# multimodallearning/convexAdam

Measured on AMD Instinct MI355X. Metric: volume-pairs/sec (160x192x224 MIND convex+Adam(80it)), higher is better.
Workload: dtype f32

## Files before the change

convexadam_amd/csrc/adam.hip:

```cpp
#include <math.h>

#include "cvx_common.h"

namespace cvx {

constexpr int BT_Z = 8, BT_Y = 8, BT_X = 32, BT_NT = 512, BT_PX = 48;

template <int PASS, bool BACKWARD, bool ADAM>
__device__ __forceinline__ void box_pass(const float* __restrict__ src, int sy, float* __restrict__ dst, int dz, int dy,
                                         int gz0, int gy0, int x0, int h, int w, int d, float* __restrict__ gout,
                                         float* __restrict__ P, float* __restrict__ m, float* __restrict__ v, AdamConsts ac,
                                         float* __restrict__ gsave) {
    constexpr int NP = 20 - PASS, C0 = 4 + PASS, SH = PASS - 1;
    const int nr = dz * dy * NP;
    for (int r = threadIdx.x; r < nr; r += BT_NT) {
        const int p = r % NP, row = r / NP;
        const int y = row % dy, z = row / dy;
        const int c = C0 + 2 * p;
        const float* win = src + ((z + 1) * sy + (y + 1)) * BT_PX + (c - 1 + SH);
        f32x2 s = {0.0f, 0.0f};
#pragma unroll
        for (int a = -1; a <= 1; ++a)
#pragma unroll
            for (int b = -1; b <= 1; ++b) {
// ... 86 lines not shown
__global__ __launch_bounds__(256) void k_adam_update(const float* __restrict__ G, float* __restrict__ P, float* __restrict__ m,
                                                     float* __restrict__ v, size_t n, AdamConsts ac) {
    const size_t i = (size_t)blockIdx.x * blockDim.x + threadIdx.x;
    if (i >= n) return;
    const float g = G[i];
    const float mo = m[i];
    const float mm = __builtin_fmaf(ac.w1, g - mo, mo);
    float vv = v[i] * ac.b2;
    vv = __builtin_fmaf(ac.omb2 * g, g, vv);
    const float den = fdiv(adam_sqrt(vv, ac.sqrt_tbl), ac.bc2s) + 1e-8f;
    P[i] = P[i] + fdiv(ac.neg_step * mm, den);
    m[i] = mm;
    v[i] = vv;
}

static int launch_box3x3(const float* in, float* out, int h, int w, int d, bool backward, float* P, float* m, float* v,
                         AdamConsts ac, float* gsave, hipStream_t s) {
    const bool force_tiled = options().box_tiled != 0;
    if (!force_tiled && (backward ? (out || P) && box3_tile_supported(in, out, h, w, d, P, m, v, gsave) : box3_tile_fwd_supported(in, out, h, w, d))) {
        long long ft = backward ? options().box_bwd_tile : options().box_fwd_tile;
        if (ft < 0) ft = box3_march_supported(d) ? box3_tile_fwd_auto(h, w, d) : 2000;
        if (ft >= 1000) return launch_box3_tile(in, out, h, w, d, (int)ft, backward, P, m, v, ac, gsave, s);
    }
    if (!force_tiled && box3_march_supported(d)) return launch_box3_march(in, out, h, w, d, backward, P, m, v, ac, gsave, s);
    const int nb = cdiv(d, BT_X) * cdiv(w, BT_Y) * cdiv(h, BT_Z) * 3;
    if (!backward) hipLaunchKernelGGL((k_box3x3<false, false>), dim3(nb), dim3(BT_NT), 0, s, in, out, h, w, d, P, m, v, ac, gsave);
    else if (!P) hipLaunchKernelGGL((k_box3x3<true, false>), dim3(nb), dim3(BT_NT), 0, s, in, out, h, w, d, P, m, v, ac, gsave);
    else hipLaunchKernelGGL((k_box3x3<true, true>), dim3(nb), dim3(BT_NT), 0, s, in, out, h, w, d, P, m, v, ac, gsave);
    return check_last("box3x3");
}

}

using namespace cvx;

extern "C" size_t cvx_adam_workspace_bytes(int C, int h, int w, int d) {
    const size_t V = (size_t)h * w * d, CP = (size_t)(C + 3) / 4 * 4;
    return 3 * (256 + sizeof(float) * 3 * V) + 2 * (256 + sizeof(float) * CP * (V + 1)) + 256;
// ... 103 lines not shown
    }

    const float nH = (float)((int64_t)3 * (h - 1) * w * d), nW = (float)((int64_t)3 * h * (w - 1) * d),
                nD = (float)((int64_t)3 * h * w * (d - 1));
    const float cH = lambda_weight / nH, cW = lambda_weight / nW, cD = lambda_weight / nD;
    const float gsc = ((1.0f / (float)V) * cost_scale) / (float)C;
    int snap = 0;
    for (int it = 0; it < niter; ++it) {
        int rc;
        const int step = step0 + it + 1;
        const double beta1 = 0.9, beta2 = 0.999;
        const double bc1 = 1.0 - pow(beta1, (double)step), bc2 = 1.0 - pow(beta2, (double)step);
        const AdamConsts ac = {(float)(1.0 - beta1), (float)beta2, (float)(1.0 - beta2), (float)sqrt(bc2), (float)(-(1.0 / bc1)), adam_sqrt_table()};
        if (fast == 2 && fused) { if ((rc = launch_box3_fast(P, U, h, w, d, nullptr, nullptr, nullptr, 1.0, 1.0, nullptr, s))) return rc; }
        else if (fast == 2 && sm->kind == 0) { if ((rc = launch_boxchain_fast(P, U, h, w, d, *sm, false, s))) return rc; }
        else if (fused) { if ((rc = launch_box3x3(P, U, h, w, d, false, nullptr, nullptr, nullptr, ac, nullptr, s))) return rc; }
        else if ((rc = launch_smoother(P, U, t1, 3, h, w, d, *sm, false, s))) return rc;
        profile_mark_kernel("adam.forward_boxes", s);
        const bool last = it == niter - 1;
        if (!(last && !keep_state && !grad_out)) {
        float* gsave = (grad_out && it == niter - 1) ? grad_out : nullptr;
        if (fast) {
            if ((rc = launch_warp_grad_fast(Fcl, Mcl, C, h, w, d, U, base_h, base_w, base_d, gsc, cH, cW, cD, gU, f16_features, s))) return rc;
            profile_mark_kernel("adam.warp_gradient", s);
            if (fused) { if ((rc = launch_box3_fast(gU, nullptr, h, w, d, P, m, v, bc1, bc2, gsave, s))) return rc; }
            else {
                if (sm->kind == 0) { if ((rc = launch_boxchain_fast(gU, t2, h, w, d, *sm, true, s))) return rc; }
                else if ((rc = launch_smoother(gU, t2, t1, 3, h, w, d, *sm, true, s))) return rc;
                if ((rc = launch_adam_update_fast(t2, P, m, v, 3 * V, bc1, bc2, s))) return rc;
                if (gsave) (void)hipMemcpyAsync(gsave, t2, sizeof(float) * 3 * V, hipMemcpyDeviceToDevice, s);
            }
        } else {
        if ((rc = launch_warp_grad(Fcl, Mcl, C, h, w, d, U, base_h, base_w, base_d, gsc, cH, cW, cD, gU, f16_features, s))) return rc;
        profile_mark_kernel("adam.warp_gradient", s);
        if (fused) { if ((rc = launch_box3x3(gU, nullptr, h, w, d, true, P, m, v, ac, gsave, s))) return rc; }
        else {
            if ((rc = launch_smoother(gU, t2, t1, 3, h, w, d, *sm, true, s))) return rc;
            hipLaunchKernelGGL(k_adam_update, dim3((unsigned)cdiv64((int64_t)(3 * V), 256)), dim3(256), 0, s, t2, P, m, v, 3 * V, ac);
            if (gsave) (void)hipMemcpyAsync(gsave, t2, sizeof(float) * 3 * V, hipMemcpyDeviceToDevice, s);
        }
        }
        }
        if (!(last && !keep_state && !grad_out)) profile_mark_kernel("adam.adjoint_update", s);
        while (snap < n_snap && snapshot_iters_host[snap] == it + 1) {
            (void)hipMemcpyAsync(snapshots + (size_t)snap * 3 * V, U, sizeof(float) * 3 * V, hipMemcpyDeviceToDevice, s);
            ++snap;
        }
    }
    return check_last("adam_run");
}
// ... 1 lines not shown
```

convexadam_amd/csrc/api.hip:

```cpp
#include <math.h>
#include <stdlib.h>
#include <string.h>
#include <new>

#include "cvx_common.h"

namespace cvx {

static thread_local char g_err[512] = "";

void set_error(const char* fmt, ...) {
    va_list ap;
    va_start(ap, fmt);
    vsnprintf(g_err, sizeof(g_err), fmt, ap);
    va_end(ap);
}
int fail(int code, const char* fmt, ...) {
    va_list ap;
    va_start(ap, fmt);
    vsnprintf(g_err, sizeof(g_err), fmt, ap);
    va_end(ap);
    return code;
}
int check_last(const char* what) {
// ... 9 lines not shown

}
struct cvx_context {
    cvx::Options opt;
    unsigned* sqrt_tbl = nullptr;
    unsigned char* exp_tbl = nullptr;
    unsigned exp_first = 0, exp_count = 0;
    int tbl_device = -1;
};
namespace cvx {
static Options env_options() {
    return {env_ll("CVX_MIND_TILED", 0),   env_ll("CVX_MIND_OVERLAP", 0),  env_ll("CVX_MM_TX", 0),        env_ll("CVX_MM_SLOTS", 512),          env_ll("CVX_BOX_TILED", 0),
            env_ll("CVX_NO_PRUNE", 0),     env_ll("CVX_CORR_UNFUSED", 0), env_ll("CVX_CORR_FUSED_ALL", 0), env_ll("CVX_PRUNE_STREAM_ABOVE", -1), env_ll("CVX_CF_CENSUS", 0), env_ll("CVX_CF_PRIO", 136),
            env_ll("CVX_WARP_FLAT", 0),    env_ll("CVX_BOX_YT", 8),       env_ll("CVX_BOX_WG_TARGET", 0),
            env_ll("CVX_BOX_XSPLIT", -1),  env_ll("CVX_BOX_CPT", 4),      env_ll("CVX_BOX_UNEVEN", 200), env_ll("CVX_BOX_ADAM_ROLE", 0), env_ll("CVX_BOX_DPP", 0),      env_ll("CVX_BOX_PK", 0),       env_ll("CVX_BOX_PRIO", 0),     env_ll("CVX_LABEL_POW_BLOCK", 32), 0,                             env_ll("CVX_MIND_MEAN_THREADS", 0),
            env_ll("CVX_EDT_SEQUENTIAL", 0), env_ll("CVX_WARP_OCTANT", 4), env_ll("CVX_BOX_FWD_TILE", -1), env_ll("CVX_BOX_BWD_TILE", -1), env_ll("CVX_BOX_WALK", 1), env_ll("CVX_CORR_DUAL", 0), env_ll("CVX_PRUNE_REFINE", 1), env_ll("CVX_MIND_RECORDS", 1), env_ll("CVX_RESIZE_UP2", 1), env_ll("CVX_MIND_BLOCKED", 1), env_ll("CVX_CORR_CERT", 1), env_ll("CVX_CC_DEBUG", 0), env_ll("CVX_IC_FUSED", 0), env_ll("CVX_MIND_SINGLE", 0), env_ll("CVX_MS_ZLEN", 0), env_ll("CVX_CF_MAP", 1), env_ll("CVX_CERT_UNFUSED", 0), env_ll("CVX_FBOX_TILE", 0)};
}
static cvx_context& default_context() {
    static cvx_context c = [] { cvx_context d; d.opt = env_options(); return d; }();
    return c;
}
static thread_local cvx_context* t_bound = nullptr;
static cvx_context& current_context() { return t_bound ? *t_bound : default_context(); }
Options& options() { return current_context().opt; }
const unsigned* adam_sqrt_table() { return current_context().sqrt_tbl; }
ExpTable mind_exp_table() {
    const cvx_context& c = current_context();
    return {c.exp_tbl, c.exp_first, c.exp_tbl ? c.exp_count : 0u};
}
ContextScope::ContextScope(const cvx_context* c) : prev_(t_bound), active_(c != nullptr) {
    if (active_) t_bound = const_cast<cvx_context*>(c);
// ... 31 lines not shown
    *slot = p;
    return CVX_OK;
}
constexpr size_t kSqrtTableBytes = ((size_t)(1u << 24) + (1u << 23)) / 4;

__global__ __launch_bounds__(256) void k_expf(const float* __restrict__ x, float* __restrict__ out, size_t n) {
    for (size_t i = (size_t)blockIdx.x * blockDim.x + threadIdx.x; i < n; i += (size_t)gridDim.x * blockDim.x) out[i] = cvx_expf(x[i]);
}
struct OptName { const char* name; long long Options::*field; };
static const OptName kOptNames[] = {{"mind_tiled", &Options::mind_tiled},     {"mind_overlap", &Options::mind_overlap},   {"mm_tx", &Options::mm_tx},
                                    {"mm_slots", &Options::mm_slots},         {"box_tiled", &Options::box_tiled},
                                    {"no_prune", &Options::no_prune},         {"corr_unfused", &Options::corr_unfused}, {"corr_fused_all", &Options::corr_fused_all},
                                    {"prune_stream_above", &Options::prune_stream_above}, {"cf_census", &Options::cf_census}, {"cf_prio", &Options::cf_prio},
                                    {"warp_flat", &Options::warp_flat},       {"box_yt", &Options::box_yt},             {"box_wg_target", &Options::box_wg_target},
                                    {"box_xsplit", &Options::box_xsplit},     {"box_cpt", &Options::box_cpt},           {"box_uneven", &Options::box_uneven},     {"box_adam_role", &Options::box_adam_role}, {"box_dpp", &Options::box_dpp},           {"box_pk", &Options::box_pk},             {"box_prio", &Options::box_prio},         {"label_pow_block", &Options::label_pow_block}, {"census_ptr", &Options::census_ptr},     {"mind_mean_threads", &Options::mind_mean_threads},
                                    {"edt_sequential", &Options::edt_sequential}, {"warp_octant", &Options::warp_octant}, {"box_fwd_tile", &Options::box_fwd_tile}, {"box_bwd_tile", &Options::box_bwd_tile}, {"box_walk", &Options::box_walk}, {"corr_dual", &Options::corr_dual}, {"prune_refine", &Options::prune_refine}, {"mind_records", &Options::mind_records}, {"resize_up2", &Options::resize_up2}, {"mind_blocked", &Options::mind_blocked}, {"corr_cert", &Options::corr_cert}, {"cc_debug", &Options::cc_debug}, {"ic_fused", &Options::ic_fused}, {"mind_single", &Options::mind_single}, {"ms_zlen", &Options::ms_zlen}, {"cf_map", &Options::cf_map}, {"cert_unfused", &Options::cert_unfused}, {"fbox_tile", &Options::fbox_tile}};

}

static int set_option_of(cvx_context& c, const char* name, long long value) {
    for (const auto& o : cvx::kOptNames)
        if (name && strcmp(name, o.name) == 0) {
            if (strcmp(name, "box_xsplit") == 0 && value > 32) return cvx::fail(CVX_ERR_INVALID_ARG, "box_xsplit %lld: at most 32 x tiles", value);
            c.opt.*(o.field) = value;
            return CVX_OK;
        }
    return cvx::fail(CVX_ERR_INVALID_ARG, "cvx_set_option: unknown option '%s'", name ? name : "(null)");
}
static long long get_option_of(const cvx_context& c, const char* name) {
    for (const auto& o : cvx::kOptNames)
        if (name && strcmp(name, o.name) == 0) return c.opt.*(o.field);
// ... 89 lines not shown
```

convexadam_amd/csrc/boxtile.hip:

```cpp
#include "cvx_common.h"

namespace cvx {

namespace {

constexpr unsigned BT_OOB = 0x80000000u;

struct BTWin { float w[3][6]; };

template <bool F, bool M, bool P>
__device__ __forceinline__ void bt_accum(const BTWin& t, float (&mid)[4], float (&pre)[4], float (&fin)[4]) {
    float f[4], m[4], p[4];
#pragma unroll
    for (int j = 0; j < 4; ++j) { f[j] = mid[j]; m[j] = pre[j]; p[j] = 0.0f; }
#pragma unroll
    for (int i = 0; i < 3; ++i)
#pragma unroll
        for (int j = 0; j < 4; ++j) {
            if (F) { f[j] += t.w[i][j]; f[j] += t.w[i][j + 1]; f[j] += t.w[i][j + 2]; }
            if (M) { m[j] += t.w[i][j]; m[j] += t.w[i][j + 1]; m[j] += t.w[i][j + 2]; }
            if (P) { p[j] += t.w[i][j]; p[j] += t.w[i][j + 1]; p[j] += t.w[i][j + 2]; }
        }
#pragma unroll
    for (int j = 0; j < 4; ++j) { fin[j] = f[j]; mid[j] = m[j]; pre[j] = p[j]; }
// ... 35 lines not shown
        bt_accum<true, false, false>(A, mid, pre, fin);
        emit(L - 1, fin);
    } else {
        load(L + 1, B);
        prep(A);
        bt_accum<true, true, false>(A, mid, pre, fin);
        emit(L - 2, fin);
        prep(B);
        bt_accum<true, false, false>(B, mid, pre, fin);
        emit(L - 1, fin);
    }
}

}

template <int TZ, int TY, int TXQ, int NW, int WPS, bool BACKWARD, bool ADAM>
__global__ __launch_bounds__(64 * NW, WPS) void k_box3_tile(const float* __restrict__ in, float* __restrict__ out, int h, int w, int d,
                                                           int ntz, int nty, int ntx, int ntiles, int NS1, int NS2, int NS3, FastDiv dvz, FastDiv dvx, FastDiv dvy,
                                                           FastDiv dn1, FastDiv dn2, FastDiv dn3, float* __restrict__ P, float* __restrict__ m, float* __restrict__ v, AdamConsts ac,
                                                           float* __restrict__ gsave) {
    constexpr int TX = 4 * TXQ, RS = TX + 4;
    constexpr int Z1 = TZ + 4, Y1 = TY + 4, Z2 = TZ + 2, Y2 = TY + 2;
    constexpr int SLOTS = NW * 4;
    static_assert(TXQ + 2 <= 16, "a row of quads must fit 16 lanes");
    __shared__ __attribute__((aligned(16))) float S[Z1 * Y1 * RS + Z2 * Y2 * RS + 8];
    float* S1 = S;
    float* S2 = S + Z1 * Y1 * RS;
    const int per_xcd = (int)(gridDim.x >> 3);
    const int bid = __builtin_amdgcn_readfirstlane((int)blockIdx.x);
    const int b = (bid & 7) * per_xcd + (bid >> 3);
    if (b >= ntiles) return;
// ... 18 lines not shown
            const int yy = gy - 1 + i;
            ro[i] = (qin && yy >= 0 && yy < w) ? (unsigned)(yy * d + gx) * 4u : BT_OOB;
        }
        const int zin0 = z0 - 3 + p0;
        auto load = [&](int n, BTWin& t) {
            const int z = zin0 + n;
            const bool zok = z >= 0 && z < h;
            const unsigned zo = (unsigned)(zok ? z : 0) * (unsigned)wd * 4u;
#pragma unroll
            for (int i = 0; i < 3; ++i) {
                const float4 a = buffer_load16(ir, (zok && ro[i] != BT_OOB) ? ro[i] + zo : BT_OOB, 0);
                t.w[i][1] = a.x; t.w[i][2] = a.y; t.w[i][3] = a.z; t.w[i][4] = a.w;
            }
        };
        auto prep = [&](BTWin& t) {
            if (BACKWARD) {
#pragma unroll
                for (int i = 0; i < 3; ++i)
#pragma unroll
                    for (int j = 1; j <= 4; ++j) t.w[i][j] = t.w[i][j] == 0.0f ? t.w[i][j] : div_exact<27>(t.w[i][j]);
            }
#pragma unroll
            for (int i = 0; i < 3; ++i) {
                t.w[i][0] = __int_as_float(__builtin_amdgcn_update_dpp(0, __float_as_int(t.w[i][4]), 0x111, 0xf, 0xf, true));
                t.w[i][5] = __int_as_float(__builtin_amdgcn_update_dpp(0, __float_as_int(t.w[i][1]), 0x101, 0xf, 0xf, true));
            }
        };
        const bool rowin = qin && gy >= 0 && gy < w;
        float* dst = S1 + (p0 * Y1 + r) * RS + 4 * q - 2;
        auto emit = [&](int k, const float (&fin)[4]) {
            const int z = z0 - 2 + p0 + k;
// ... 55 lines not shown
                for (int i = 0; i < 3; ++i) {
                    const float* rp = src + (n * Y2 + i) * RS;
                    const f32x4 a = lds_load4(rp);
                    const f32x2 e = lds_load2(rp + 4);
                    t.w[i][0] = a.x; t.w[i][1] = a.y; t.w[i][2] = a.z; t.w[i][3] = a.w; t.w[i][4] = e.x; t.w[i][5] = e.y;
                }
            };
            const size_t o0 = ((size_t)(z0 + p0) * w + gy) * d + gx;
            auto emit = [&](int k, const float (&fin)[4]) {
                if (z0 + p0 + k >= h) return;
                const size_t o = o0 + (size_t)k * wd;
                if (!BACKWARD) {
                    *reinterpret_cast<float4*>(oc + o) = make_float4(div_exact<27>(fin[0]), div_exact<27>(fin[1]), div_exact<27>(fin[2]), div_exact<27>(fin[3]));
                } else if (!ADAM) {
                    *reinterpret_cast<float4*>(oc + o) = make_float4(fin[0], fin[1], fin[2], fin[3]);
                } else {
                    float* Pc = P + (size_t)c * V + o; float* mc = m + (size_t)c * V + o; float* vc = v + (size_t)c * V + o;
                    const float4 p4 = *reinterpret_cast<const float4*>(Pc), m4 = *reinterpret_cast<const float4*>(mc), v4 = *reinterpret_cast<const float4*>(vc);
                    float pp[4] = {p4.x, p4.y, p4.z, p4.w}, mm[4] = {m4.x, m4.y, m4.z, m4.w}, vv[4] = {v4.x, v4.y, v4.z, v4.w};
#pragma unroll
                    for (int j = 0; j < 4; ++j) adam_update(fin[j], pp[j], mm[j], vv[j], ac);
                    *reinterpret_cast<float4*>(Pc) = make_float4(pp[0], pp[1], pp[2], pp[3]);
                    *reinterpret_cast<float4*>(mc) = make_float4(mm[0], mm[1], mm[2], mm[3]);
                    *reinterpret_cast<float4*>(vc) = make_float4(vv[0], vv[1], vv[2], vv[3]);
                    if (gsave) *reinterpret_cast<float4*>(gsave + (size_t)c * V + o) = make_float4(fin[0], fin[1], fin[2], fin[3]);
                }
            };
            bt_walk(L, load, [](BTWin&) {}, emit);
        }
    }
}

bool box3_tile_supported(const float* in, const float* out, int h, int w, int d, const float* P, const float* m, const float* v, const float* gsave) {
    auto al = [](const void* p) { return (reinterpret_cast<uintptr_t>(p) & 15) == 0; };
    return (d % 4 == 0) && al(in) && al(out) && al(P) && al(m) && al(v) && al(gsave) && in != out && (size_t)h * w * d * 4 < ((size_t)1 << 31);
}
bool box3_tile_fwd_supported(const float* in, const float* out, int h, int w, int d) { return out && box3_tile_supported(in, out, h, w, d, nullptr, nullptr, nullptr, nullptr); }

template <int TZ, int TY, int TXQ, int NW, int WPS>
static int launch_tile_t(const float* in, float* out, int h, int w, int d, int ns1, int ns2, int ns3, bool backward, float* P, float* m, float* v,
                         AdamConsts ac, float* gsave, hipStream_t s) {
    const int ntz = cdiv(h, TZ), nty = cdiv(w, TY), ntx = cdiv(d, 4 * TXQ);
    const int ntiles = 3 * ntz * nty * ntx;
    const unsigned nb = (unsigned)((ntiles + 7) / 8 * 8);
    auto clampns = [](int ns, int planes) { return ns < 1 ? 1 : (ns > planes / 2 ? planes / 2 : ns); };
    const int a1 = clampns(ns1, TZ + 4), a2 = clampns(ns2, TZ + 2), a3 = clampns(ns3, TZ);
#define CVX_BT_LAUNCH(B, A) hipLaunchKernelGGL((k_box3_tile<TZ, TY, TXQ, NW, WPS, B, A>), dim3(nb), dim3(64 * NW), 0, s, in, out, h, w, d, ntz, nty, ntx, ntiles, a1, a2, a3, fastdiv_make(ntz), fastdiv_make(ntx), fastdiv_make(nty), fastdiv_make(a1), fastdiv_make(a2), fastdiv_make(a3), P, m, v, ac, gsave)
    if (!backward) CVX_BT_LAUNCH(false, false);
    else if (!P) CVX_BT_LAUNCH(true, false);
    else CVX_BT_LAUNCH(true, true);
#undef CVX_BT_LAUNCH
    return check_last("box3_tile");
}

int launch_box3_tile(const float* in, float* out, int h, int w, int d, int variant, bool backward, float* P, float* m, float* v, AdamConsts ac,
                     float* gsave, hipStream_t s) {
    const int kind = variant / 1000, ns = variant % 1000;
    int ns1 = ns / 100, ns2 = (ns / 10) % 10, ns3 = ns % 10;
    if (kind == 1) {
        if (!ns) { ns1 = 5; ns2 = 3; ns3 = 4; }
        return launch_tile_t<12, 8, 14, 8, 4>(in, out, h, w, d, ns1, ns2, ns3, backward, P, m, v, ac, gsave, s);
    }
    if (!ns) { ns1 = 4; ns2 = 3; ns3 = 4; }
    return launch_tile_t<12, 16, 14, 16, 4>(in, out, h, w, d, ns1, ns2, ns3, backward, P, m, v, ac, gsave, s);
}
int launch_box3_tile_fwd(const float* in, float* out, int h, int w, int d, int variant, hipStream_t s) {
    return launch_box3_tile(in, out, h, w, d, variant, false, nullptr, nullptr, nullptr, AdamConsts{}, nullptr, s);
}

int box3_tile_fwd_auto(int h, int w, int d) {
    const int n2 = 3 * cdiv(h, 12) * cdiv(w, 16) * cdiv(d, 56);
    return n2 >= 192 ? 2000 : 0;
}

}
```

convexadam_amd/csrc/cvx_common.h:

```cpp
#pragma once
#include <hip/hip_runtime.h>
#include <stdint.h>
#include <stdio.h>
#include <stdarg.h>

#include <mutex>

#include "convexadam_hip.h"

namespace cvx {

void set_error(const char* fmt, ...);
int fail(int code, const char* fmt, ...);
int check_last(const char* what);

#define CVX_REQUIRE(cond, ...)                                      \
    do {                                                            \
        if (!(cond)) return ::cvx::fail(CVX_ERR_INVALID_ARG, __VA_ARGS__); \
    } while (0)

static inline hipStream_t as_stream(void* s) { return reinterpret_cast<hipStream_t>(s); }
static inline size_t align_up(size_t v, size_t a) { return (v + a - 1) / a * a; }
static inline int cdiv(int a, int b) { return (a + b - 1) / b; }
static inline int64_t cdiv64(int64_t a, int64_t b) { return (a + b - 1) / b; }
// ... 54 lines not shown
    long long box_bwd_tile;
    long long box_walk;
    long long corr_dual;
    long long prune_refine;
    long long mind_records;
    long long resize_up2;
    long long mind_blocked;
    long long corr_cert;
    long long cc_debug;
    long long ic_fused;
    long long mind_single;
    long long ms_zlen;
    long long cf_map;
    long long cert_unfused;
    long long fbox_tile;
};
Options& options();
const unsigned* adam_sqrt_table();
class ContextScope {
public:
    explicit ContextScope(const cvx_context* c);
    ~ContextScope();
    ContextScope(const ContextScope&) = delete;
    ContextScope& operator=(const ContextScope&) = delete;
private:
    void* prev_;
    bool active_;
};

#ifdef CVX_RACE_JITTER
// ... 231 lines not shown
size_t corr_certify_workspace_bytes(int C, int h, int w, int d, int hw, bool plain = false);
int corr_certified_argmin(const float* ssdu, const float* fix, const float* mov, int C, int h, int w, int d, int hw, int64_t* argmin,
                          void* workspace, size_t workspace_bytes, hipStream_t s);
int coupled_convex_cert_impl(const float* ssduA, const float* fixA, const float* movA, float* outA, void* wsA, const float* ssduB, const float* fixB,
                             const float* movB, float* outB, void* wsB, const float* mesh, int C, int h, int w, int d, int hw, size_t workspace_bytes,
                             hipStream_t s, int stage = 0);
bool corr_use_unfused(int C, int h, int w, int d, int hw, bool variant);
bool box3_march_supported(int d);
int launch_box3_march(const float* in, float* out, int h, int w, int d, bool backward, float* P, float* m, float* v,
                      AdamConsts ac, float* gsave, hipStream_t s);
bool box3_tile_fwd_supported(const float* in, const float* out, int h, int w, int d);
int launch_box3_tile_fwd(const float* in, float* out, int h, int w, int d, int variant, hipStream_t s);
int box3_tile_fwd_auto(int h, int w, int d);
bool box3_tile_supported(const float* in, const float* out, int h, int w, int d, const float* P, const float* m, const float* v, const float* gsave);
int launch_box3_tile(const float* in, float* out, int h, int w, int d, int variant, bool backward, float* P, float* m, float* v, AdamConsts ac,
                     float* gsave, hipStream_t s);
int launch_to_chunked(const float* in, int C, size_t V, float* out, bool half, hipStream_t s);
int launch_warp_grad(const float* Fcl, const float* Mcl, int C, int h, int w, int d, const float* U, const float* bh,
                     const float* bw, const float* bd, float gsc, float cH, float cW, float cD, float* gU, bool half, hipStream_t s);
int launch_warp_grad_fast(const float* Fcl, const float* Mcl, int C, int h, int w, int d, const float* U, const float* bh,
                          const float* bw, const float* bd, float gsc, float cH, float cW, float cD, float* gU, bool half, hipStream_t s);
int launch_box3_fast(const float* in, float* out, int h, int w, int d, float* P, float* m, float* v, double bc1, double bc2,
                     float* gsave, hipStream_t s);
bool boxchain_fast_supported(const cvx_smoother& sm, int h, int w, int d);
int launch_boxchain_fast(const float* in, float* out, int h, int w, int d, const cvx_smoother& sm, bool reverse, hipStream_t s);
int launch_adam_update_fast(const float* G, float* P, float* m, float* v, size_t n, double bc1, double bc2, hipStream_t s);

}
```

convexadam_amd/csrc/warp.hip:

```cpp
#include "cvx_common.h"

namespace cvx {

__global__ __launch_bounds__(256) void k_to_chunked(const float* __restrict__ in, int C, size_t V, float* __restrict__ out) {
    const size_t p = (size_t)blockIdx.x * blockDim.x + threadIdx.x;
    if (p > V) return;
    const int c0 = 4 * (int)blockIdx.y;
    float4 r = make_float4(0.f, 0.f, 0.f, 0.f);
    if (p < V) {
        const float* src = in + (size_t)c0 * V + p;
        r.x = src[0];
        if (c0 + 1 < C) r.y = src[V];
        if (c0 + 2 < C) r.z = src[2 * V];
        if (c0 + 3 < C) r.w = src[3 * V];
    }
    reinterpret_cast<float4*>(out)[(size_t)blockIdx.y * (V + 1) + p] = r;
}

typedef _Float16 h16x4 __attribute__((ext_vector_type(4)));
__global__ __launch_bounds__(256) void k_to_chunked_h(const float* __restrict__ in, int C, size_t V, uint2* __restrict__ out) {
    const size_t p = (size_t)blockIdx.x * blockDim.x + threadIdx.x;
    if (p > V) return;
    const int c0 = 4 * (int)blockIdx.y;
    float4 r = make_float4(0.f, 0.f, 0.f, 0.f);
    if (p < V) {
        const float* src = in + (size_t)c0 * V + p;
        r.x = src[0];
        if (c0 + 1 < C) r.y = src[V];
        if (c0 + 2 < C) r.z = src[2 * V];
        if (c0 + 3 < C) r.w = src[3 * V];
    }
    const h16x4 o = {(_Float16)r.x, (_Float16)r.y, (_Float16)r.z, (_Float16)r.w};
    out[(size_t)blockIdx.y * (V + 1) + p] = __builtin_bit_cast(uint2, o);
}
__device__ __forceinline__ float4 buffer_load8h(__amdgpu_buffer_rsrc_t rsrc, unsigned lane_off, unsigned uni_off) {
    const h16x4 v = __builtin_bit_cast(h16x4, __builtin_amdgcn_raw_buffer_load_b64(rsrc, (int)lane_off, (int)uni_off, 0));
    return make_float4((float)v.x, (float)v.y, (float)v.z, (float)v.w);
}

template <bool BUF, bool HALF = false>
__global__ __launch_bounds__(256) void k_warp_grad(const float* __restrict__ F2, const float* __restrict__ M2, int C, int CP,
                                                   int h, int w, int d, const float* __restrict__ U,
                                                   const float* __restrict__ bh, const float* __restrict__ bw,
                                                   const float* __restrict__ bd, float gsc, float cH, float cW, float cD,
                                                   float* __restrict__ gU, unsigned long long* __restrict__ census, FastDiv dx, FastDiv dy,
                                                   float sc0, float sc1, float sc2) {
    const size_t V = (size_t)h * w * d;
    if (census && threadIdx.x == 0) {
        census[4 * blockIdx.x] = __builtin_amdgcn_s_memrealtime();
        census[4 * blockIdx.x + 3] = __builtin_amdgcn_s_getreg((4 << 0) | (0 << 6) | (31 << 11)) | ((unsigned long long)__builtin_amdgcn_s_getreg((20 << 0) | (0 << 6) | (31 << 11)) << 32);
    }
    const int ntx = (d + 15) / 16, nty = (w + 3) / 4, ntz = (h + 3) / 4;
    const int per_xcd = (int)(gridDim.x >> 3);
    const int bid = __builtin_amdgcn_readfirstlane((int)blockIdx.x);
    const int tile = (bid & 7) * per_xcd + (bid >> 3);
// ... 16 lines not shown
    unsigned off[8];
    off[0] = (zin0 && yin0 && xin0) ? (unsigned)(r00 + x0) * REC : zero_rec; off[1] = (zin0 && yin0 && xin1) ? (unsigned)(r00 + x1) * REC : zero_rec;
    off[2] = (zin0 && yin1 && xin0) ? (unsigned)(r01 + x0) * REC : zero_rec; off[3] = (zin0 && yin1 && xin1) ? (unsigned)(r01 + x1) * REC : zero_rec;
    off[4] = (zin1 && yin0 && xin0) ? (unsigned)(r10 + x0) * REC : zero_rec; off[5] = (zin1 && yin0 && xin1) ? (unsigned)(r10 + x1) * REC : zero_rec;
    off[6] = (zin1 && yin1 && xin0) ? (unsigned)(r11 + x0) * REC : zero_rec; off[7] = (zin1 && yin1 && xin1) ? (unsigned)(r11 + x1) * REC : zero_rec;
    const float wgt[8] = {t.tnw, t.tne, t.tsw, t.tse, t.bnw, t.bne, t.bsw, t.bse};
    const float ax[8] = {fy1 - t.iy, fy1 - t.iy, t.iy - fy0, t.iy - fy0, fy1 - t.iy, fy1 - t.iy, t.iy - fy0, t.iy - fy0};
    const float bx[8] = {fz1 - t.iz, fz1 - t.iz, fz1 - t.iz, fz1 - t.iz, t.iz - fz0, t.iz - fz0, t.iz - fz0, t.iz - fz0};
    const float ay[8] = {fx1 - t.ix, t.ix - fx0, fx1 - t.ix, t.ix - fx0, fx1 - t.ix, t.ix - fx0, fx1 - t.ix, t.ix - fx0};
    const float bz[8] = {fy1 - t.iy, fy1 - t.iy, t.iy - fy0, t.iy - fy0, fy1 - t.iy, fy1 - t.iy, t.iy - fy0, t.iy - fy0};
    float gix = 0.f, giy = 0.f, giz = 0.f;
    const unsigned foff = p * REC;
    const unsigned chunk_bytes = (unsigned)(V + 1) * REC;
    const __amdgpu_buffer_rsrc_t mr = __builtin_amdgcn_make_buffer_rsrc(const_cast<float*>(M2), 0, (int)(chunk_bytes * (unsigned)(CP / 4)), 0x00020000);
    const __amdgpu_buffer_rsrc_t fr = __builtin_amdgcn_make_buffer_rsrc(const_cast<float*>(F2), 0, (int)(chunk_bytes * (unsigned)(CP / 4)), 0x00020000);
    unsigned coff = 0;
    for (int c0 = 0; c0 < CP / 4; ++c0, coff += chunk_bytes) {
        float vv[8][4], fv[4];
#pragma unroll
        for (int k = 0; k < 8; ++k) {
            const float4 q = HALF ? buffer_load8h(mr, off[k], coff) : BUF ? buffer_load16(mr, off[k], coff) : *reinterpret_cast<const float4*>(reinterpret_cast<const char*>(M2) + (size_t)c0 * chunk_bytes + off[k]);
            vv[k][0] = q.x; vv[k][1] = q.y; vv[k][2] = q.z; vv[k][3] = q.w;
        }
        const float4 fq = HALF ? buffer_load8h(fr, foff, coff) : BUF ? buffer_load16(fr, foff, coff) : *reinterpret_cast<const float4*>(reinterpret_cast<const char*>(F2) + (size_t)c0 * chunk_bytes + foff);
        fv[0] = fq.x; fv[1] = fq.y; fv[2] = fq.z; fv[3] = fq.w;
#pragma unroll
        for (int j = 0; j < 4; ++j) {
            float wv = 0.0f;
#pragma unroll
            for (int k = 0; k < 8; ++k) wv += vv[k][j] * wgt[k];
// ... 1 lines not shown
            const float gOut = gsc * (2.0f * df);
            gix -= vv[0][j] * ax[0] * bx[0] * gOut; giy -= vv[0][j] * ay[0] * bx[0] * gOut; giz -= vv[0][j] * ay[0] * bz[0] * gOut;
            gix += vv[1][j] * ax[1] * bx[1] * gOut; giy -= vv[1][j] * ay[1] * bx[1] * gOut; giz -= vv[1][j] * ay[1] * bz[1] * gOut;
            gix -= vv[2][j] * ax[2] * bx[2] * gOut; giy += vv[2][j] * ay[2] * bx[2] * gOut; giz -= vv[2][j] * ay[2] * bz[2] * gOut;
            gix += vv[3][j] * ax[3] * bx[3] * gOut; giy += vv[3][j] * ay[3] * bx[3] * gOut; giz -= vv[3][j] * ay[3] * bz[3] * gOut;
            gix -= vv[4][j] * ax[4] * bx[4] * gOut; giy -= vv[4][j] * ay[4] * bx[4] * gOut; giz += vv[4][j] * ay[4] * bz[4] * gOut;
            gix += vv[5][j] * ax[5] * bx[5] * gOut; giy -= vv[5][j] * ay[5] * bx[5] * gOut; giz += vv[5][j] * ay[5] * bz[5] * gOut;
            gix -= vv[6][j] * ax[6] * bx[6] * gOut; giy += vv[6][j] * ay[6] * bx[6] * gOut; giz += vv[6][j] * ay[6] * bz[6] * gOut;
            gix += vv[7][j] * ax[7] * bx[7] * gOut; giy += vv[7][j] * ay[7] * bx[7] * gOut; giz += vv[7][j] * ay[7] * bz[7] * gOut;
        }
    }
    float g[3];
    g[0] = fdiv(((float)h / 2.0f) * giz, sc0);
    g[1] = fdiv(((float)w / 2.0f) * giy, sc1);
    g[2] = fdiv(((float)d / 2.0f) * gix, sc2);
    const unsigned sH = (unsigned)(w * d);
    const unsigned pxp = x < d - 1 ? p + 1 : p, pxm = x > 0 ? p - 1 : p, pzp = z < h - 1 ? p + sH : p, pzm = z > 0 ? p - sH : p,
                   pyp = y < w - 1 ? p + (unsigned)d : p, pym = y > 0 ? p - (unsigned)d : p;
    float nb[3][6];
    const __amdgpu_buffer_rsrc_t ur = __builtin_amdgcn_make_buffer_rsrc(const_cast<float*>(U), 0, (int)(12u * (unsigned)V), 0x00020000);
    const unsigned nboff[6] = {4u * pxp, 4u * pxm, 4u * pzp, 4u * pzm, 4u * pyp, 4u * pym};
#pragma unroll
    for (int a = 0; a < 3; ++a)
#pragma unroll
        for (int k = 0; k < 6; ++k) nb[a][k] = __builtin_bit_cast(float, __builtin_amdgcn_raw_buffer_load_b32(ur, (int)nboff[k], (int)(4u * (unsigned)V) * a, 0));
    const float uc3[3] = {uH, uW, uD};
#pragma unroll
    for (int a = 0; a < 3; ++a) {
        const float uc = uc3[a];
        float acc = g[a], t;
        t = acc + -(cD * (2.0f * (nb[a][0] - uc))); acc = x < d - 1 ? t : acc;
        t = acc +  (cD * (2.0f * (uc - nb[a][1]))); acc = x > 0 ? t : acc;
        t = acc + -(cH * (2.0f * (nb[a][2] - uc))); acc = z < h - 1 ? t : acc;
        t = acc +  (cH * (2.0f * (uc - nb[a][3]))); acc = z > 0 ? t : acc;
        t = acc + -(cW * (2.0f * (nb[a][4] - uc))); acc = y < w - 1 ? t : acc;
        t = acc +  (cW * (2.0f * (uc - nb[a][5]))); acc = y > 0 ? t : acc;
        (gU + (size_t)a * V)[p] = acc;
    }
    if (census && threadIdx.x == 0) census[4 * blockIdx.x + 2] = __builtin_amdgcn_s_memrealtime();
}


int launch_to_chunked(const float* in, int C, size_t V, float* out, bool half, hipStream_t s) {
    const int CP = (C + 3) / 4 * 4;
    if ((size_t)(CP / 4) * (V + 1) * 16 >= ((size_t)1 << 31)) return fail(CVX_ERR_UNSUPPORTED, "adam_run: control grid too large (%zu voxels x %d channels)", V, C);
    if (half) hipLaunchKernelGGL(k_to_chunked_h, dim3((unsigned)cdiv64((int64_t)(V + 1), 256), CP / 4), dim3(256), 0, s, in, C, V, reinterpret_cast<uint2*>(out));
    else hipLaunchKernelGGL(k_to_chunked, dim3((unsigned)cdiv64((int64_t)(V + 1), 256), CP / 4), dim3(256), 0, s, in, C, V, out);
    return check_last("to_chunked");
}

int launch_warp_grad(const float* Fcl, const float* Mcl, int C, int h, int w, int d, const float* U, const float* bh,
                     const float* bw, const float* bd, float gsc, float cH, float cW, float cD, float* gU, bool half, hipStream_t s) {
    const int CP = (C + 3) / 4 * 4;
    const dim3 gv((unsigned)((cdiv(d, 16) * cdiv(w, 4) * cdiv(h, 4) + 7) / 8 * 8));
    unsigned long long* census = reinterpret_cast<unsigned long long*>(options().census_ptr);
    if (census) census += 8 * 1024;
    const FastDiv dx = fastdiv_make(cdiv(d, 16)), dy = fastdiv_make(cdiv(w, 4));
    const float sc0 = (float)((h - 1) / 2.0), sc1 = (float)((w - 1) / 2.0), sc2 = (float)((d - 1) / 2.0);
    if (half) hipLaunchKernelGGL((k_warp_grad<true, true>), gv, dim3(256), 0, s, Fcl, Mcl, C, CP, h, w, d, U, bh, bw, bd, gsc, cH, cW, cD, gU, census, dx, dy, sc0, sc1, sc2);
    else if (options().warp_flat) hipLaunchKernelGGL(k_warp_grad<false>, gv, dim3(256), 0, s, Fcl, Mcl, C, CP, h, w, d, U, bh, bw, bd, gsc, cH, cW, cD, gU, census, dx, dy, sc0, sc1, sc2);
    else hipLaunchKernelGGL(k_warp_grad<true>, gv, dim3(256), 0, s, Fcl, Mcl, C, CP, h, w, d, U, bh, bw, bd, gsc, cH, cW, cD, gU, census, dx, dy, sc0, sc1, sc2);
    return check_last("warp_grad");
}

}
```

Before: 147.8.

## Pre-divide adjoint taps in warp grad, phase Adam update, hoist neighbour loads

The warp-gradient kernel can now write gradients already divided by 27, so the backward box-tile kernel skips its per-window division prep step. The tile kernel gains a PHASE mode that stages the smoothed gradient in LDS, then does the Adam update after a barrier with batched buffer loads of P/m/v. A third option issues the six-neighbour displacement loads before the channel loop to hide their latency. All three are on by default through new options, at the cost of more template variants, an extra barrier, and higher register pressure from the early loads.

Result: no change. 148.2 (median of 6 runs) (+0.3%).

```diff
diff --git a/convexadam_amd/csrc/adam.hip b/convexadam_amd/csrc/adam.hip
--- a/convexadam_amd/csrc/adam.hip
+++ b/convexadam_amd/csrc/adam.hip
@@ -124,14 +124,20 @@
     v[i] = vv;
 }
 
+static int box3x3_tile_variant(const float* in, const float* out, int h, int w, int d, bool backward, const float* P, const float* m, const float* v,
+                               const float* gsave) {
+    if (options().box_tiled != 0) return 0;
+    if (!(backward ? (out || P) && box3_tile_supported(in, out, h, w, d, P, m, v, gsave) : box3_tile_fwd_supported(in, out, h, w, d))) return 0;
+    long long ft = backward ? options().box_bwd_tile : options().box_fwd_tile;
+    if (ft < 0) ft = box3_march_supported(d) ? box3_tile_fwd_auto(h, w, d) : 2000;
+    return ft >= 1000 ? (int)ft : 0;
+}
+
 static int launch_box3x3(const float* in, float* out, int h, int w, int d, bool backward, float* P, float* m, float* v,
-                         AdamConsts ac, float* gsave, hipStream_t s) {
+                         AdamConsts ac, float* gsave, bool prediv, hipStream_t s) {
     const bool force_tiled = options().box_tiled != 0;
-    if (!force_tiled && (backward ? (out || P) && box3_tile_supported(in, out, h, w, d, P, m, v, gsave) : box3_tile_fwd_supported(in, out, h, w, d))) {
-        long long ft = backward ? options().box_bwd_tile : options().box_fwd_tile;
-        if (ft < 0) ft = box3_march_supported(d) ? box3_tile_fwd_auto(h, w, d) : 2000;
-        if (ft >= 1000) return launch_box3_tile(in, out, h, w, d, (int)ft, backward, P, m, v, ac, gsave, s);
-    }
+    if (const int ft = box3x3_tile_variant(in, out, h, w, d, backward, P, m, v, gsave)) return launch_box3_tile(in, out, h, w, d, ft, backward, P, m, v, ac, gsave, prediv, s);
+    if (prediv) return fail(CVX_ERR_UNSUPPORTED, "box3x3: pre-divided adjoint taps need the tile kernel");
     if (!force_tiled && box3_march_supported(d)) return launch_box3_march(in, out, h, w, d, backward, P, m, v, ac, gsave, s);
     const int nb = cdiv(d, BT_X) * cdiv(w, BT_Y) * cdiv(h, BT_Z) * 3;
     if (!backward) hipLaunchKernelGGL((k_box3x3<false, false>), dim3(nb), dim3(BT_NT), 0, s, in, out, h, w, d, P, m, v, ac, gsave);
@@ -265,7 +271,7 @@
         const AdamConsts ac = {(float)(1.0 - beta1), (float)beta2, (float)(1.0 - beta2), (float)sqrt(bc2), (float)(-(1.0 / bc1)), adam_sqrt_table()};
         if (fast == 2 && fused) { if ((rc = launch_box3_fast(P, U, h, w, d, nullptr, nullptr, nullptr, 1.0, 1.0, nullptr, s))) return rc; }
         else if (fast == 2 && sm->kind == 0) { if ((rc = launch_boxchain_fast(P, U, h, w, d, *sm, false, s))) return rc; }
-        else if (fused) { if ((rc = launch_box3x3(P, U, h, w, d, false, nullptr, nullptr, nullptr, ac, nullptr, s))) return rc; }
+        else if (fused) { if ((rc = launch_box3x3(P, U, h, w, d, false, nullptr, nullptr, nullptr, ac, nullptr, false, s))) return rc; }
         else if ((rc = launch_smoother(P, U, t1, 3, h, w, d, *sm, false, s))) return rc;
         profile_mark_kernel("adam.forward_boxes", s);
         const bool last = it == niter - 1;
@@ -282,9 +288,10 @@
                 if (gsave) (void)hipMemcpyAsync(gsave, t2, sizeof(float) * 3 * V, hipMemcpyDeviceToDevice, s);
             }
         } else {
-        if ((rc = launch_warp_grad(Fcl, Mcl, C, h, w, d, U, base_h, base_w, base_d, gsc, cH, cW, cD, gU, f16_features, s))) return rc;
+        const bool prediv = fused && options().warp_prediv && box3x3_tile_variant(gU, nullptr, h, w, d, true, P, m, v, gsave) != 0;
+        if ((rc = launch_warp_grad(Fcl, Mcl, C, h, w, d, U, base_h, base_w, base_d, gsc, cH, cW, cD, gU, f16_features, prediv, s))) return rc;
         profile_mark_kernel("adam.warp_gradient", s);
-        if (fused) { if ((rc = launch_box3x3(gU, nullptr, h, w, d, true, P, m, v, ac, gsave, s))) return rc; }
+        if (fused) { if ((rc = launch_box3x3(gU, nullptr, h, w, d, true, P, m, v, ac, gsave, prediv, s))) return rc; }
         else {
             if ((rc = launch_smoother(gU, t2, t1, 3, h, w, d, *sm, true, s))) return rc;
             hipLaunchKernelGGL(k_adam_update, dim3((unsigned)cdiv64((int64_t)(3 * V), 256)), dim3(256), 0, s, t2, P, m, v, 3 * V, ac);
diff --git a/convexadam_amd/csrc/api.hip b/convexadam_amd/csrc/api.hip
--- a/convexadam_amd/csrc/api.hip
+++ b/convexadam_amd/csrc/api.hip
@@ -47,7 +47,8 @@
             env_ll("CVX_NO_PRUNE", 0),     env_ll("CVX_CORR_UNFUSED", 0), env_ll("CVX_CORR_FUSED_ALL", 0), env_ll("CVX_PRUNE_STREAM_ABOVE", -1), env_ll("CVX_CF_CENSUS", 0), env_ll("CVX_CF_PRIO", 136),
             env_ll("CVX_WARP_FLAT", 0),    env_ll("CVX_BOX_YT", 8),       env_ll("CVX_BOX_WG_TARGET", 0),
             env_ll("CVX_BOX_XSPLIT", -1),  env_ll("CVX_BOX_CPT", 4),      env_ll("CVX_BOX_UNEVEN", 200), env_ll("CVX_BOX_ADAM_ROLE", 0), env_ll("CVX_BOX_DPP", 0),      env_ll("CVX_BOX_PK", 0),       env_ll("CVX_BOX_PRIO", 0),     env_ll("CVX_LABEL_POW_BLOCK", 32), 0,                             env_ll("CVX_MIND_MEAN_THREADS", 0),
-            env_ll("CVX_EDT_SEQUENTIAL", 0), env_ll("CVX_WARP_OCTANT", 4), env_ll("CVX_BOX_FWD_TILE", -1), env_ll("CVX_BOX_BWD_TILE", -1), env_ll("CVX_BOX_WALK", 1), env_ll("CVX_CORR_DUAL", 0), env_ll("CVX_PRUNE_REFINE", 1), env_ll("CVX_MIND_RECORDS", 1), env_ll("CVX_RESIZE_UP2", 1), env_ll("CVX_MIND_BLOCKED", 1), env_ll("CVX_CORR_CERT", 1), env_ll("CVX_CC_DEBUG", 0), env_ll("CVX_IC_FUSED", 0), env_ll("CVX_MIND_SINGLE", 0), env_ll("CVX_MS_ZLEN", 0), env_ll("CVX_CF_MAP", 1), env_ll("CVX_CERT_UNFUSED", 0), env_ll("CVX_FBOX_TILE", 0)};
+            env_ll("CVX_EDT_SEQUENTIAL", 0), env_ll("CVX_WARP_OCTANT", 4), env_ll("CVX_BOX_FWD_TILE", -1), env_ll("CVX_BOX_BWD_TILE", -1), env_ll("CVX_BOX_WALK", 1), env_ll("CVX_CORR_DUAL", 0), env_ll("CVX_PRUNE_REFINE", 1), env_ll("CVX_MIND_RECORDS", 1), env_ll("CVX_RESIZE_UP2", 1), env_ll("CVX_MIND_BLOCKED", 1), env_ll("CVX_CORR_CERT", 1), env_ll("CVX_CC_DEBUG", 0), env_ll("CVX_IC_FUSED", 0), env_ll("CVX_MIND_SINGLE", 0), env_ll("CVX_MS_ZLEN", 0), env_ll("CVX_CF_MAP", 1), env_ll("CVX_CERT_UNFUSED", 0), env_ll("CVX_FBOX_TILE", 0),
+            env_ll("CVX_WARP_PREDIV", 1), env_ll("CVX_BOX_ADAM_PHASE", 1), env_ll("CVX_WARP_EARLY_NB", 1)};
 }
 static cvx_context& default_context() {
     static cvx_context c = [] { cvx_context d; d.opt = env_options(); return d; }();
@@ -109,7 +110,8 @@
                                     {"prune_stream_above", &Options::prune_stream_above}, {"cf_census", &Options::cf_census}, {"cf_prio", &Options::cf_prio},
                                     {"warp_flat", &Options::warp_flat},       {"box_yt", &Options::box_yt},             {"box_wg_target", &Options::box_wg_target},
                                     {"box_xsplit", &Options::box_xsplit},     {"box_cpt", &Options::box_cpt},           {"box_uneven", &Options::box_uneven},     {"box_adam_role", &Options::box_adam_role}, {"box_dpp", &Options::box_dpp},           {"box_pk", &Options::box_pk},             {"box_prio", &Options::box_prio},         {"label_pow_block", &Options::label_pow_block}, {"census_ptr", &Options::census_ptr},     {"mind_mean_threads", &Options::mind_mean_threads},
-                                    {"edt_sequential", &Options::edt_sequential}, {"warp_octant", &Options::warp_octant}, {"box_fwd_tile", &Options::box_fwd_tile}, {"box_bwd_tile", &Options::box_bwd_tile}, {"box_walk", &Options::box_walk}, {"corr_dual", &Options::corr_dual}, {"prune_refine", &Options::prune_refine}, {"mind_records", &Options::mind_records}, {"resize_up2", &Options::resize_up2}, {"mind_blocked", &Options::mind_blocked}, {"corr_cert", &Options::corr_cert}, {"cc_debug", &Options::cc_debug}, {"ic_fused", &Options::ic_fused}, {"mind_single", &Options::mind_single}, {"ms_zlen", &Options::ms_zlen}, {"cf_map", &Options::cf_map}, {"cert_unfused", &Options::cert_unfused}, {"fbox_tile", &Options::fbox_tile}};
+                                    {"edt_sequential", &Options::edt_sequential}, {"warp_octant", &Options::warp_octant}, {"box_fwd_tile", &Options::box_fwd_tile}, {"box_bwd_tile", &Options::box_bwd_tile}, {"box_walk", &Options::box_walk}, {"corr_dual", &Options::corr_dual}, {"prune_refine", &Options::prune_refine}, {"mind_records", &Options::mind_records}, {"resize_up2", &Options::resize_up2}, {"mind_blocked", &Options::mind_blocked}, {"corr_cert", &Options::corr_cert}, {"cc_debug", &Options::cc_debug}, {"ic_fused", &Options::ic_fused}, {"mind_single", &Options::mind_single}, {"ms_zlen", &Options::ms_zlen}, {"cf_map", &Options::cf_map}, {"cert_unfused", &Options::cert_unfused}, {"fbox_tile", &Options::fbox_tile},
+                                    {"warp_prediv", &Options::warp_prediv}, {"box_adam_phase", &Options::box_adam_phase}, {"warp_early_nb", &Options::warp_early_nb}};
 
 }
 
diff --git a/convexadam_amd/csrc/boxtile.hip b/convexadam_amd/csrc/boxtile.hip
--- a/convexadam_amd/csrc/boxtile.hip
+++ b/convexadam_amd/csrc/boxtile.hip
@@ -73,7 +73,7 @@
 
 }
 
-template <int TZ, int TY, int TXQ, int NW, int WPS, bool BACKWARD, bool ADAM>
+template <int TZ, int TY, int TXQ, int NW, int WPS, bool BACKWARD, bool ADAM, bool PREDIV = false, bool PHASE = false>
 __global__ __launch_bounds__(64 * NW, WPS) void k_box3_tile(const float* __restrict__ in, float* __restrict__ out, int h, int w, int d,
                                                            int ntz, int nty, int ntx, int ntiles, int NS1, int NS2, int NS3, FastDiv dvz, FastDiv dvx, FastDiv dvy,
                                                            FastDiv dn1, FastDiv dn2, FastDiv dn3, float* __restrict__ P, float* __restrict__ m, float* __restrict__ v, AdamConsts ac,
@@ -122,7 +122,7 @@
             }
         };
         auto prep = [&](BTWin& t) {
-            if (BACKWARD) {
+            if (BACKWARD && !PREDIV) {
 #pragma unroll
                 for (int i = 0; i < 3; ++i)
 #pragma unroll
@@ -208,6 +208,8 @@
                     *reinterpret_cast<float4*>(oc + o) = make_float4(div_exact<27>(fin[0]), div_exact<27>(fin[1]), div_exact<27>(fin[2]), div_exact<27>(fin[3]));
                 } else if (!ADAM) {
                     *reinterpret_cast<float4*>(oc + o) = make_float4(fin[0], fin[1], fin[2], fin[3]);
+                } else if (PHASE) {
+                    lds_store4(S1 + ((p0 + k) * TY + r) * TX + 4 * q, f32x4{fin[0], fin[1], fin[2], fin[3]});
                 } else {
                     float* Pc = P + (size_t)c * V + o; float* mc = m + (size_t)c * V + o; float* vc = v + (size_t)c * V + o;
                     const float4 p4 = *reinterpret_cast<const float4*>(Pc), m4 = *reinterpret_cast<const float4*>(mc), v4 = *reinterpret_cast<const float4*>(vc);
@@ -223,6 +225,40 @@
             bt_walk(L, load, [](BTWin&) {}, emit);
         }
     }
+    if constexpr (ADAM && PHASE) {
+        static_assert(TZ * TY * TX <= Z1 * Y1 * RS, "the G tile must fit the stage-1 region");
+        constexpr int NQ = TZ * TY * TXQ, NT = 64 * NW, QPT = (NQ + NT - 1) / NT;
+        cvx_barrier();
+        const unsigned vb = (unsigned)(V * sizeof(float));
+        const __amdgpu_buffer_rsrc_t pr = __builtin_amdgcn_make_buffer_rsrc(P + (size_t)c * V, 0, (int)vb, 0x00020000);
+        const __amdgpu_buffer_rsrc_t mr = __builtin_amdgcn_make_buffer_rsrc(m + (size_t)c * V, 0, (int)vb, 0x00020000);
+        const __amdgpu_buffer_rsrc_t vr = __builtin_amdgcn_make_buffer_rsrc(v + (size_t)c * V, 0, (int)vb, 0x00020000);
+        unsigned go[QPT];
+        float4 p4[QPT], m4[QPT], v4[QPT];
+#pragma unroll
+        for (int i = 0; i < QPT; ++i) {
+            const int qi = tid + i * NT;
+            const int zz = qi / (TY * TXQ), yy = (qi / TXQ) % TY, xq = qi % TXQ;
+            const int gz = z0 + zz, gy = y0 + yy, gx = x0 + 4 * xq;
+            go[i] = (qi < NQ && gz < h && gy < w && gx < d) ? (unsigned)((gz * w + gy) * d + gx) * 4u : BT_OOB;
+        }
+#pragma unroll
+        for (int i = 0; i < QPT; ++i) { p4[i] = buffer_load16(pr, go[i], 0); m4[i] = buffer_load16(mr, go[i], 0); v4[i] = buffer_load16(vr, go[i], 0); }
+#pragma unroll
+        for (int i = 0; i < QPT; ++i) {
+            if (go[i] == BT_OOB) continue;
+            const f32x4 g4 = lds_load4(S1 + 4 * (tid + i * NT));
+            const float gg[4] = {g4.x, g4.y, g4.z, g4.w};
+            float pp[4] = {p4[i].x, p4[i].y, p4[i].z, p4[i].w}, mm[4] = {m4[i].x, m4[i].y, m4[i].z, m4[i].w}, vv[4] = {v4[i].x, v4[i].y, v4[i].z, v4[i].w};
+#pragma unroll
+            for (int j = 0; j < 4; ++j) adam_update(gg[j], pp[j], mm[j], vv[j], ac);
+            const size_t o = (size_t)c * V + go[i] / 4u;
+            *reinterpret_cast<float4*>(P + o) = make_float4(pp[0], pp[1], pp[2], pp[3]);
+            *reinterpret_cast<float4*>(m + o) = make_float4(mm[0], mm[1], mm[2], mm[3]);
+            *reinterpret_cast<float4*>(v + o) = make_float4(vv[0], vv[1], vv[2], vv[3]);
+            if (gsave) *reinterpret_cast<float4*>(gsave + o) = make_float4(gg[0], gg[1], gg[2], gg[3]);
+        }
+    }
 }
 
 bool box3_tile_supported(const float* in, const float* out, int h, int w, int d, const float* P, const float* m, const float* v, const float* gsave) {
@@ -233,33 +269,35 @@
 
 template <int TZ, int TY, int TXQ, int NW, int WPS>
 static int launch_tile_t(const float* in, float* out, int h, int w, int d, int ns1, int ns2, int ns3, bool backward, float* P, float* m, float* v,
-                         AdamConsts ac, float* gsave, hipStream_t s) {
+                         AdamConsts ac, float* gsave, bool prediv, hipStream_t s) {
     const int ntz = cdiv(h, TZ), nty = cdiv(w, TY), ntx = cdiv(d, 4 * TXQ);
     const int ntiles = 3 * ntz * nty * ntx;
     const unsigned nb = (unsigned)((ntiles + 7) / 8 * 8);
     auto clampns = [](int ns, int planes) { return ns < 1 ? 1 : (ns > planes / 2 ? planes / 2 : ns); };
     const int a1 = clampns(ns1, TZ + 4), a2 = clampns(ns2, TZ + 2), a3 = clampns(ns3, TZ);
-#define CVX_BT_LAUNCH(B, A) hipLaunchKernelGGL((k_box3_tile<TZ, TY, TXQ, NW, WPS, B, A>), dim3(nb), dim3(64 * NW), 0, s, in, out, h, w, d, ntz, nty, ntx, ntiles, a1, a2, a3, fastdiv_make(ntz), fastdiv_make(ntx), fastdiv_make(nty), fastdiv_make(a1), fastdiv_make(a2), fastdiv_make(a3), P, m, v, ac, gsave)
+#define CVX_BT_LAUNCH(...) hipLaunchKernelGGL((k_box3_tile<TZ, TY, TXQ, NW, WPS, __VA_ARGS__>), dim3(nb), dim3(64 * NW), 0, s, in, out, h, w, d, ntz, nty, ntx, ntiles, a1, a2, a3, fastdiv_make(ntz), fastdiv_make(ntx), fastdiv_make(nty), fastdiv_make(a1), fastdiv_make(a2), fastdiv_make(a3), P, m, v, ac, gsave)
+    const bool phase = options().box_adam_phase != 0;
     if (!backward) CVX_BT_LAUNCH(false, false);
-    else if (!P) CVX_BT_LAUNCH(true, false);
-    else CVX_BT_LAUNCH(true, true);
+    else if (!P) { if (prediv) CVX_BT_LAUNCH(true, false, true); else CVX_BT_LAUNCH(true, false); }
+    else if (prediv) { if (phase) CVX_BT_LAUNCH(true, true, true, true); else CVX_BT_LAUNCH(true, true, true, false); }
+    else { if (phase) CVX_BT_LAUNCH(true, true, false, true); else CVX_BT_LAUNCH(true, true, false, false); }
 #undef CVX_BT_LAUNCH
     return check_last("box3_tile");
 }
 
 int launch_box3_tile(const float* in, float* out, int h, int w, int d, int variant, bool backward, float* P, float* m, float* v, AdamConsts ac,
-                     float* gsave, hipStream_t s) {
+                     float* gsave, bool prediv, hipStream_t s) {
     const int kind = variant / 1000, ns = variant % 1000;
     int ns1 = ns / 100, ns2 = (ns / 10) % 10, ns3 = ns % 10;
     if (kind == 1) {
         if (!ns) { ns1 = 5; ns2 = 3; ns3 = 4; }
-        return launch_tile_t<12, 8, 14, 8, 4>(in, out, h, w, d, ns1, ns2, ns3, backward, P, m, v, ac, gsave, s);
+        return launch_tile_t<12, 8, 14, 8, 4>(in, out, h, w, d, ns1, ns2, ns3, backward, P, m, v, ac, gsave, prediv, s);
     }
     if (!ns) { ns1 = 4; ns2 = 3; ns3 = 4; }
-    return launch_tile_t<12, 16, 14, 16, 4>(in, out, h, w, d, ns1, ns2, ns3, backward, P, m, v, ac, gsave, s);
+    return launch_tile_t<12, 16, 14, 16, 4>(in, out, h, w, d, ns1, ns2, ns3, backward, P, m, v, ac, gsave, prediv, s);
 }
 int launch_box3_tile_fwd(const float* in, float* out, int h, int w, int d, int variant, hipStream_t s) {
-    return launch_box3_tile(in, out, h, w, d, variant, false, nullptr, nullptr, nullptr, AdamConsts{}, nullptr, s);
+    return launch_box3_tile(in, out, h, w, d, variant, false, nullptr, nullptr, nullptr, AdamConsts{}, nullptr, false, s);
 }
 
 int box3_tile_fwd_auto(int h, int w, int d) {
diff --git a/convexadam_amd/csrc/cvx_common.h b/convexadam_amd/csrc/cvx_common.h
--- a/convexadam_amd/csrc/cvx_common.h
+++ b/convexadam_amd/csrc/cvx_common.h
@@ -92,6 +92,9 @@
     long long cf_map;
     long long cert_unfused;
     long long fbox_tile;
+    long long warp_prediv;
+    long long box_adam_phase;
+    long long warp_early_nb;
 };
 Options& options();
 const unsigned* adam_sqrt_table();
@@ -353,10 +356,10 @@
 int box3_tile_fwd_auto(int h, int w, int d);
 bool box3_tile_supported(const float* in, const float* out, int h, int w, int d, const float* P, const float* m, const float* v, const float* gsave);
 int launch_box3_tile(const float* in, float* out, int h, int w, int d, int variant, bool backward, float* P, float* m, float* v, AdamConsts ac,
-                     float* gsave, hipStream_t s);
+                     float* gsave, bool prediv, hipStream_t s);
 int launch_to_chunked(const float* in, int C, size_t V, float* out, bool half, hipStream_t s);
 int launch_warp_grad(const float* Fcl, const float* Mcl, int C, int h, int w, int d, const float* U, const float* bh,
-                     const float* bw, const float* bd, float gsc, float cH, float cW, float cD, float* gU, bool half, hipStream_t s);
+                     const float* bw, const float* bd, float gsc, float cH, float cW, float cD, float* gU, bool half, bool prediv, hipStream_t s);
 int launch_warp_grad_fast(const float* Fcl, const float* Mcl, int C, int h, int w, int d, const float* U, const float* bh,
                           const float* bw, const float* bd, float gsc, float cH, float cW, float cD, float* gU, bool half, hipStream_t s);
 int launch_box3_fast(const float* in, float* out, int h, int w, int d, float* P, float* m, float* v, double bc1, double bc2,
diff --git a/convexadam_amd/csrc/warp.hip b/convexadam_amd/csrc/warp.hip
--- a/convexadam_amd/csrc/warp.hip
+++ b/convexadam_amd/csrc/warp.hip
@@ -38,7 +38,7 @@
     return make_float4((float)v.x, (float)v.y, (float)v.z, (float)v.w);
 }
 
-template <bool BUF, bool HALF = false>
+template <bool BUF, bool HALF = false, bool PREDIV = false, bool EARLY_NB = false>
 __global__ __launch_bounds__(256) void k_warp_grad(const float* __restrict__ F2, const float* __restrict__ M2, int C, int CP,
                                                    int h, int w, int d, const float* __restrict__ U,
                                                    const float* __restrict__ bh, const float* __restrict__ bw,
@@ -85,6 +85,19 @@
     const unsigned chunk_bytes = (unsigned)(V + 1) * REC;
     const __amdgpu_buffer_rsrc_t mr = __builtin_amdgcn_make_buffer_rsrc(const_cast<float*>(M2), 0, (int)(chunk_bytes * (unsigned)(CP / 4)), 0x00020000);
     const __amdgpu_buffer_rsrc_t fr = __builtin_amdgcn_make_buffer_rsrc(const_cast<float*>(F2), 0, (int)(chunk_bytes * (unsigned)(CP / 4)), 0x00020000);
+    const unsigned sH = (unsigned)(w * d);
+    const unsigned pxp = x < d - 1 ? p + 1 : p, pxm = x > 0 ? p - 1 : p, pzp = z < h - 1 ? p + sH : p, pzm = z > 0 ? p - sH : p,
+                   pyp = y < w - 1 ? p + (unsigned)d : p, pym = y > 0 ? p - (unsigned)d : p;
+    float nb[3][6];
+    const __amdgpu_buffer_rsrc_t ur = __builtin_amdgcn_make_buffer_rsrc(const_cast<float*>(U), 0, (int)(12u * (unsigned)V), 0x00020000);
+    const unsigned nboff[6] = {4u * pxp, 4u * pxm, 4u * pzp, 4u * pzm, 4u * pyp, 4u * pym};
+    auto load_nb = [&]() {
+#pragma unroll
+        for (int a = 0; a < 3; ++a)
+#pragma unroll
+            for (int k = 0; k < 6; ++k) nb[a][k] = __builtin_bit_cast(float, __builtin_amdgcn_raw_buffer_load_b32(ur, (int)nboff[k], (int)(4u * (unsigned)V) * a, 0));
+    };
+    if (EARLY_NB) load_nb();
     unsigned coff = 0;
     for (int c0 = 0; c0 < CP / 4; ++c0, coff += chunk_bytes) {
         float vv[8][4], fv[4];
@@ -116,16 +129,7 @@
     g[0] = fdiv(((float)h / 2.0f) * giz, sc0);
     g[1] = fdiv(((float)w / 2.0f) * giy, sc1);
     g[2] = fdiv(((float)d / 2.0f) * gix, sc2);
-    const unsigned sH = (unsigned)(w * d);
-    const unsigned pxp = x < d - 1 ? p + 1 : p, pxm = x > 0 ? p - 1 : p, pzp = z < h - 1 ? p + sH : p, pzm = z > 0 ? p - sH : p,
-                   pyp = y < w - 1 ? p + (unsigned)d : p, pym = y > 0 ? p - (unsigned)d : p;
-    float nb[3][6];
-    const __amdgpu_buffer_rsrc_t ur = __builtin_amdgcn_make_buffer_rsrc(const_cast<float*>(U), 0, (int)(12u * (unsigned)V), 0x00020000);
-    const unsigned nboff[6] = {4u * pxp, 4u * pxm, 4u * pzp, 4u * pzm, 4u * pyp, 4u * pym};
-#pragma unroll
-    for (int a = 0; a < 3; ++a)
-#pragma unroll
-        for (int k = 0; k < 6; ++k) nb[a][k] = __builtin_bit_cast(float, __builtin_amdgcn_raw_buffer_load_b32(ur, (int)nboff[k], (int)(4u * (unsigned)V) * a, 0));
+    if (!EARLY_NB) load_nb();
     const float uc3[3] = {uH, uW, uD};
 #pragma unroll
     for (int a = 0; a < 3; ++a) {
@@ -137,7 +141,7 @@
         t = acc +  (cH * (2.0f * (uc - nb[a][3]))); acc = z > 0 ? t : acc;
         t = acc + -(cW * (2.0f * (nb[a][4] - uc))); acc = y < w - 1 ? t : acc;
         t = acc +  (cW * (2.0f * (uc - nb[a][5]))); acc = y > 0 ? t : acc;
-        (gU + (size_t)a * V)[p] = acc;
+        (gU + (size_t)a * V)[p] = PREDIV ? (acc == 0.0f ? acc : div_exact<27>(acc)) : acc;
     }
     if (census && threadIdx.x == 0) census[4 * blockIdx.x + 2] = __builtin_amdgcn_s_memrealtime();
 }
@@ -152,16 +156,19 @@
 }
 
 int launch_warp_grad(const float* Fcl, const float* Mcl, int C, int h, int w, int d, const float* U, const float* bh,
-                     const float* bw, const float* bd, float gsc, float cH, float cW, float cD, float* gU, bool half, hipStream_t s) {
+                     const float* bw, const float* bd, float gsc, float cH, float cW, float cD, float* gU, bool half, bool prediv, hipStream_t s) {
     const int CP = (C + 3) / 4 * 4;
     const dim3 gv((unsigned)((cdiv(d, 16) * cdiv(w, 4) * cdiv(h, 4) + 7) / 8 * 8));
     unsigned long long* census = reinterpret_cast<unsigned long long*>(options().census_ptr);
     if (census) census += 8 * 1024;
     const FastDiv dx = fastdiv_make(cdiv(d, 16)), dy = fastdiv_make(cdiv(w, 4));
     const float sc0 = (float)((h - 1) / 2.0), sc1 = (float)((w - 1) / 2.0), sc2 = (float)((d - 1) / 2.0);
-    if (half) hipLaunchKernelGGL((k_warp_grad<true, true>), gv, dim3(256), 0, s, Fcl, Mcl, C, CP, h, w, d, U, bh, bw, bd, gsc, cH, cW, cD, gU, census, dx, dy, sc0, sc1, sc2);
-    else if (options().warp_flat) hipLaunchKernelGGL(k_warp_grad<false>, gv, dim3(256), 0, s, Fcl, Mcl, C, CP, h, w, d, U, bh, bw, bd, gsc, cH, cW, cD, gU, census, dx, dy, sc0, sc1, sc2);
-    else hipLaunchKernelGGL(k_warp_grad<true>, gv, dim3(256), 0, s, Fcl, Mcl, C, CP, h, w, d, U, bh, bw, bd, gsc, cH, cW, cD, gU, census, dx, dy, sc0, sc1, sc2);
+#define CVX_WG_LAUNCH(...) hipLaunchKernelGGL((k_warp_grad<__VA_ARGS__>), gv, dim3(256), 0, s, Fcl, Mcl, C, CP, h, w, d, U, bh, bw, bd, gsc, cH, cW, cD, gU, census, dx, dy, sc0, sc1, sc2)
+    if (half) { if (prediv) CVX_WG_LAUNCH(true, true, true); else CVX_WG_LAUNCH(true, true, false); }
+    else if (options().warp_flat) { if (prediv) CVX_WG_LAUNCH(false, false, true); else CVX_WG_LAUNCH(false, false, false); }
+    else if (options().warp_early_nb) { if (prediv) CVX_WG_LAUNCH(true, false, true, true); else CVX_WG_LAUNCH(true, false, false, true); }
+    else { if (prediv) CVX_WG_LAUNCH(true, false, true); else CVX_WG_LAUNCH(true, false, false); }
+#undef CVX_WG_LAUNCH
     return check_last("warp_grad");
 }
 
```
